# puzzlepaint/camera_calibration

Measured on AMD Instinct MI355X. Metric: M observations/sec per LM iteration, higher is better.
Workload: dtype f64

## Files before the change

camera_calibration_amd/csrc/kernels_obs.hip:

```cpp
#include "cba_internal.h"
#include <algorithm>
#include <mutex>

namespace cba {

__device__ __forceinline__ void quat_mul(const double* a, const double* b, double* o) {
  o[0] = a[0] * b[0] - a[1] * b[1] - a[2] * b[2] - a[3] * b[3];
  o[1] = a[0] * b[1] + a[1] * b[0] + a[2] * b[3] - a[3] * b[2];
  o[2] = a[0] * b[2] + a[2] * b[0] + a[3] * b[1] - a[1] * b[3];
  o[3] = a[0] * b[3] + a[3] * b[0] + a[1] * b[2] - a[2] * b[1];
}
__device__ __forceinline__ void quat_rotate(const double* q, const double* v, double* o) {
  double ux = 2 * (q[2] * v[2] - q[3] * v[1]);
  double uy = 2 * (q[3] * v[0] - q[1] * v[2]);
  double uz = 2 * (q[1] * v[1] - q[2] * v[0]);
  o[0] = v[0] + q[0] * ux + (q[2] * uz - q[3] * uy);
  o[1] = v[1] + q[0] * uy + (q[3] * ux - q[1] * uz);
  o[2] = v[2] + q[0] * uz + (q[1] * uy - q[2] * ux);
}
__device__ __forceinline__ void quat_to_matrix(const double* q, double* R) {
  double tx = 2 * q[1], ty = 2 * q[2], tz = 2 * q[3];
  double twx = tx * q[0], twy = ty * q[0], twz = tz * q[0];
  double txx = tx * q[1], txy = ty * q[1], txz = tz * q[1];
  double tyy = ty * q[2], tyz = tz * q[2], tzz = tz * q[3];
// ... 722 lines not shown
  cells[2 * o] = (int)floor(gx) - 1;
  cells[2 * o + 1] = (int)floor(gy) - 1;
  flags[o] = 3;
  return !localize_only;
}
__global__ void __launch_bounds__(256) k_assemble(PassArgs a, int rig_in_state, int localize_only,
                                                  const double* __restrict__ rig7, const double* __restrict__ camrig7,
                                                  int tasks_per_obs, int rec_doubles, const double* __restrict__ pixels,
                                                  uint8_t* __restrict__ flags, const double* __restrict__ fd_out,
                                                  const uint8_t* __restrict__ fd_ok, double* __restrict__ jrec,
                                                  int* __restrict__ cells, uint8_t* __restrict__ fd_slow) {
  const int64_t o = (int64_t)blockIdx.x * blockDim.x + threadIdx.x;
  const bool with_jacobian = assemble_header(a, o, rig_in_state, localize_only, rig7, camrig7, tasks_per_obs, rec_doubles, pixels, flags,
                                             fd_out, fd_ok, jrec, cells);
  if (o < a.n_obs) fd_slow[o] = flags[o] == 1;
  (void)with_jacobian;
}
int launch_assemble(const PassArgs& a, const Layout& L, const DevState& st, int tasks_per_obs, int rec_doubles,
                    const double* pixels, uint8_t* flags, const double* fd_out, const uint8_t* fd_ok, double* jrec,
                    int* cells, uint8_t* fd_slow, hipStream_t s) {
  if (a.n_obs == 0) return CBA_OK;
  hipLaunchKernelGGL(k_assemble, dim3((unsigned)((a.n_obs + 255) / 256)), dim3(256), 0, s, a, L.rig_in_state,
                     L.localize_only, st.rig_tr_global, st.camera_tr_rig, tasks_per_obs, rec_doubles, pixels, flags,
                     fd_out, fd_ok, jrec, cells, fd_slow);
  CBA_HIP(hipGetLastError());
  return CBA_OK;
}

struct AccumLayout {
  int rig_in_state, eliminate_points, localize_only;
  int first_rig_tr_global, first_camera_tr_rig, first_points;
  int block_dof, block_size, dense_dof;
};
static_assert(std::is_trivially_copyable_v<AccumLayout>);

constexpr int kAccChunk = 8;
constexpr int kAccChunkHot = 64;
constexpr int kHotMax = 12;
constexpr int kHotPairs = kHotMax * (kHotMax + 1) / 2;

template <bool DET> struct Acc;
template <> struct Acc<false> {
  typedef double T;
  static __device__ __forceinline__ T from(double v, double) { return v; }
  static __device__ __forceinline__ void add(double* p, T v) { unsafeAtomicAdd(p, v); }
  static __device__ __forceinline__ void add_lds(double* p, T v) { __hip_atomic_fetch_add(p, v, __ATOMIC_RELAXED, __HIP_MEMORY_SCOPE_WORKGROUP); }
  static __device__ __forceinline__ double to_double(T v, double) { return v; }
};
template <> struct Acc<true> {
  typedef long long T;
  static __device__ __forceinline__ T from(double v, double scale) { return __double2ll_rn(v * scale); }
  static __device__ __forceinline__ void add(double* p, T v) { atomicAdd(reinterpret_cast<unsigned long long*>(p), (unsigned long long)v); }
  static __device__ __forceinline__ void add_lds(double* p, T v) {
    __hip_atomic_fetch_add(reinterpret_cast<unsigned long long*>(p), (unsigned long long)v, __ATOMIC_RELAXED, __HIP_MEMORY_SCOPE_WORKGROUP);
  }
  static __device__ __forceinline__ double to_double(T v, double scale) { return (double)v / scale; }
};

template <bool DET>
__device__ __forceinline__ void acc_add_H(const AccumLayout& L, const AccumTargets& T, int row, int col, typename Acc<DET>::T v) {
  if (row < L.block_dof) {
    if (col < L.block_dof) {
      int blk = row / L.block_size;
      int base = blk * L.block_size;
      Acc<DET>::add(T.Dblk + (size_t)blk * L.block_size * L.block_size + (row - base) * L.block_size + (col - base), v);
    } else {
      Acc<DET>::add(T.B + (size_t)row * L.dense_dof + (col - L.block_dof), v);
    }
  } else {
    Acc<DET>::add(T.Hdd + (size_t)(row - L.block_dof) * L.dense_dof + (col - L.block_dof), v);
  }
}
template <bool DET>
__device__ __forceinline__ void acc_add_b(const AccumLayout& L, const AccumTargets& T, int row, typename Acc<DET>::T v) {
  if (row < L.block_dof) Acc<DET>::add(T.bblk + row, v);
  else Acc<DET>::add(T.bd + (row - L.block_dof), v);
}

template <bool DET>
__global__ void __launch_bounds__(256) k_accumulate(PassArgs a, AccumLayout L, int rec_doubles,
                                                    const uint8_t* __restrict__ flags, const double* __restrict__ jrec,
                                                    const int* __restrict__ cells, const uint32_t* __restrict__ pair_tables,
                                                    const int* __restrict__ pair_counts, AccumTargets T,
                                                    const double* __restrict__ det_scale, int points_separate) {
  typedef typename Acc<DET>::T acc_t;
  const double scale = DET ? det_scale[0] : 1.0;
  const double scale_b = DET ? det_scale[1] : 1.0;
  __shared__ double sJ0[4][kMaxCols];
  __shared__ double sJ1[4][kMaxCols];
  __shared__ double sW0[4][kMaxCols];
  __shared__ double sW1[4][kMaxCols];
  __shared__ int sIdx[4][kMaxCols];
  const int lane = threadIdx.x & 63, wv = threadIdx.x >> 6;
  const int chunk = points_separate ? kAccChunkHot : kAccChunk;
  const int64_t o_begin = ((int64_t)blockIdx.x * 4 + wv) * chunk;
  const int nrig = L.rig_in_state ? 6 : 0;
  const int nh = 6 + nrig;
  const int h0 = L.eliminate_points ? 3 : 0;
  const int nhp = nh * (nh + 1) / 2;
  int hs_i[2], hs_k[2];
#pragma unroll
  for (int t = 0; t < 2; ++t) {
    int sidx = lane + 64 * t;
    hs_i[t] = -1; hs_k[t] = -1;
    if (sidx < nhp) {
      int rem = sidx, i = 0;
      while (rem >= nh - i) { rem -= nh - i; ++i; }
      hs_i[t] = i; hs_k[t] = i + rem;
    } else if (sidx < nhp + nh) {
      hs_i[t] = sidx - nhp; hs_k[t] = -2;
    }
  }
  acc_t hot[2] = {0, 0};
  int cur_pose = -1, cur_rig = -1;
  auto flush = [&]() {
    if (cur_pose < 0) return;
#pragma unroll
    for (int t = 0; t < 2; ++t) {
      if (hs_i[t] < 0) continue;
      int row = hs_i[t] < 6 ? cur_pose + hs_i[t] : cur_rig + hs_i[t] - 6;
      if (hs_k[t] == -2) acc_add_b<DET>(L, T, row, hot[t]);
      else acc_add_H<DET>(L, T, row, hs_k[t] < 6 ? cur_pose + hs_k[t] : cur_rig + hs_k[t] - 6, hot[t]);
      hot[t] = 0;
    }
  };
  for (int c = 0; c < chunk; ++c) {
    const int64_t o = o_begin + c;
    if (o >= a.n_obs) break;
    if (flags[o] != 3) continue;
    const int cam = a.obs_camera[o];
    const CamDev cd = a.cams[cam];
    const int per = cd.params_per_point;
    const int Kg = L.localize_only ? 0 : per * 16;
    const int K = 6 + nrig + 3 + Kg;
    const double* rec = jrec + (size_t)o * rec_doubles;
    const double w = rec[2];
    const int pose_idx = L.first_rig_tr_global + 6 * (a.pose_slot ? a.pose_slot[a.obs_image[o]] : a.obs_image[o]);
    const int rig_idx = L.first_camera_tr_rig + 6 * cam;
    const int point_idx = L.first_points + 3 * a.obs_point[o];
    if (pose_idx != cur_pose || rig_idx != cur_rig) {
      flush();
      cur_pose = pose_idx; cur_rig = rig_idx;
    }
    const int cx0 = cells[2 * o], cy0 = cells[2 * o + 1];
    __builtin_amdgcn_wave_barrier();
    const int Ks = points_separate ? nh : K;
    for (int k = lane; k < Ks; k += 64) {
      int idx; double j0, j1;
      int kk = k;
      if (L.eliminate_points) {
        if (kk < 3) { idx = point_idx + kk; j0 = rec[27 + kk]; j1 = rec[30 + kk]; goto done; }
        kk -= 3;
      }
      if (kk < 6) { idx = pose_idx + kk; j0 = rec[3 + kk]; j1 = rec[9 + kk]; goto done; }
      kk -= 6;
      if (nrig) {
        if (kk < 6) { idx = rig_idx + kk; j0 = rec[15 + kk]; j1 = rec[21 + kk]; goto done; }
        kk -= 6;
      }
      if (!L.eliminate_points) {
        if (kk < 3) { idx = point_idx + kk; j0 = rec[27 + kk]; j1 = rec[30 + kk]; goto done; }
        kk -= 3;
      }
      {
        int cell = kk / per, d = kk - cell * per;
        int seq = (cx0 + (cell & 3)) + (cy0 + (cell >> 2)) * cd.gw;
        idx = L.block_dof + grid_column(cd, seq, d);
        j0 = rec[kRecHeader + kk]; j1 = rec[kRecHeader + Kg + kk];
      }
    done:
      sIdx[wv][k] = idx;
      sJ0[wv][k] = j0; sJ1[wv][k] = j1;
      sW0[wv][k] = w * j0; sW1[wv][k] = w * j1;
    }
    __builtin_amdgcn_wave_barrier();
    __builtin_amdgcn_fence(__ATOMIC_RELEASE, "wavefront");
    const double r0 = rec[0], r1 = rec[1];
#pragma unroll
    for (int t = 0; t < 2; ++t) {
      if (hs_i[t] < 0) continue;
      const int i = h0 + hs_i[t];
      if (hs_k[t] == -2) hot[t] += Acc<DET>::from(r0 * sW0[wv][i] + r1 * sW1[wv][i], scale_b);
      else { const int k = h0 + hs_k[t]; hot[t] += Acc<DET>::from(sW0[wv][i] * sJ0[wv][k] + sW1[wv][i] * sJ1[wv][k], scale); }
    }
    if (points_separate) continue;
    for (int k = lane; k < K - Kg; k += 64) {
      if (k >= h0 && k < h0 + nh) continue;
      acc_add_b<DET>(L, T, sIdx[wv][k], Acc<DET>::from(r0 * sW0[wv][k] + r1 * sW1[wv][k], scale_b));
    }
    const int slot = (per == 2) ? 0 : 1;
    const int npairs = pair_counts[slot];
    const uint32_t* table = pair_tables + (size_t)slot * (kMaxCols * (kMaxCols + 1) / 2);
    for (int e = lane; e < npairs; e += 64) {
      uint32_t pr = table[e];
      int i = pr >> 16, k = pr & 0xffff;
      double v = sW0[wv][i] * sJ0[wv][k] + sW1[wv][i] * sJ1[wv][k];
      acc_add_H<DET>(L, T, sIdx[wv][i], sIdx[wv][k], Acc<DET>::from(v, scale));
    }
  }
  flush();
}
constexpr int kPointChunkColsMax = 5120;
constexpr int kPointThreads = 1024;
constexpr int kPointUnroll = 4;
template <bool DET>
__global__ void __launch_bounds__(kPointThreads) k_accumulate_points(PassArgs a, AccumLayout L, int rec_doubles, const uint8_t* __restrict__ flags,
                                                                     const double* __restrict__ jrec, const int* __restrict__ cells,
                                                                     const int* __restrict__ key_start, const int* __restrict__ key_obs,
                                                                     int n_points, int nchunks, int chunk_cols, AccumTargets T,
                                                                     const double* __restrict__ det_scale) {
  typedef typename Acc<DET>::T acc_t;
  constexpr int NT = kPointThreads, NW = kPointThreads / 64, U = kPointUnroll;
  extern __shared__ double s_rows[];
  __shared__ acc_t s_red[NW][27];
  const double scale = DET ? det_scale[0] : 1.0;
  const double scale_b = DET ? det_scale[1] : 1.0;
  const int key = blockIdx.x / nchunks, chunk = blockIdx.x - key * nchunks;
  const int cam = key / n_points, pt = key - cam * n_points;
  const CamDev& cd = a.cams[cam];
  const int per = cd.params_per_point, gw = cd.gw;
  const int* __restrict__ gperm = cd.gperm;
  const int Kg = L.localize_only ? 0 : per * 16;
  const int ncols = Kg ? per * gw * cd.gh : 0;
  const int c0 = chunk * chunk_cols;
  const int o_begin = key_start[key], n = key_start[key + 1] - o_begin;
  if (n == 0 || (chunk > 0 && c0 >= ncols)) return;
  const int c1 = c0 + chunk_cols < ncols ? c0 + chunk_cols : ncols;
  const int tid = threadIdx.x, lane = tid & 63, wv = tid >> 6;
  const int nrig = L.rig_in_state ? 6 : 0;
  const int point_idx = L.first_points + 3 * pt;
  if (c0 < c1) {
    for (int i = tid; i < 3 * chunk_cols; i += NT) s_rows[i] = 0.0;
    __syncthreads();
    const int items = n * Kg;
    for (int it0 = tid; it0 < items; it0 += NT * U) {
      int64_t o[U]; int kk[U]; bool live[U];
#pragma unroll
      for (int u = 0; u < U; ++u) {
        const int it = it0 + u * NT;
        live[u] = it < items;
        const int oi = live[u] ? it / Kg : 0;
        kk[u] = live[u] ? it - oi * Kg : 0;
        o[u] = key_obs[o_begin + oi];
      }
      int cx[U], cy[U]; uint8_t fl[U];
#pragma unroll
      for (int u = 0; u < U; ++u) { fl[u] = flags[o[u]]; cx[u] = cells[2 * o[u]]; cy[u] = cells[2 * o[u] + 1]; }
      int col[U];
#pragma unroll
      for (int u = 0; u < U; ++u) {
        const int cell = kk[u] / per, d = kk[u] - cell * per;
        int seq = (cx[u] + (cell & 3)) + (cy[u] + (cell >> 2)) * gw;
        live[u] = live[u] && fl[u] == 3;
        if (!live[u]) seq = 0;
        col[u] = per * (gperm ? gperm[seq] : seq) + d;
        live[u] = live[u] && col[u] >= c0 && col[u] < c1;
      }
      double w[U], g0[U], g1[U], q0[U][3], q1[U][3];
#pragma unroll
      for (int u = 0; u < U; ++u) {
        if (!live[u]) continue;
        const double* rec = jrec + (size_t)o[u] * rec_doubles;
        w[u] = rec[2]; g0[u] = rec[kRecHeader + kk[u]]; g1[u] = rec[kRecHeader + Kg + kk[u]];
#pragma unroll
        for (int r = 0; r < 3; ++r) { q0[u][r] = rec[27 + r]; q1[u][r] = rec[30 + r]; }
      }
#pragma unroll
      for (int u = 0; u < U; ++u) {
        if (!live[u]) continue;
#pragma unroll
        for (int r = 0; r < 3; ++r)
          Acc<DET>::add_lds(&s_rows[r * chunk_cols + (col[u] - c0)], Acc<DET>::from((w[u] * q0[u][r]) * g0[u] + (w[u] * q1[u][r]) * g1[u], scale));
      }
    }
    __syncthreads();
#pragma unroll
    for (int r = 0; r < 3; ++r) {
      double* out = T.Hdd + (size_t)(point_idx - L.block_dof + r) * L.dense_dof + cd.intr_offset + c0;
      for (int c = tid; c < c1 - c0; c += NT) out[c] = s_rows[r * chunk_cols + c];
    }
// ... 185 lines not shown
#pragma unroll 1
    for (int r = 0; r < nrec; ++r) {
      const double w = sW[r];
      if (tid < KG) bacc += Acc<DET>::from(sRes[r][0] * (w * sJ0[r][tid]) + sRes[r][1] * (w * sJ1[r][tid]), scale_b);
      if (has_tile) {
        double a0[TZ], a1[TZ], b0[TZ], b1[TZ];
#pragma unroll
        for (int x = 0; x < TZ; ++x) { a0[x] = sJ0[r][i0 + x]; a1[x] = sJ1[r][i0 + x]; b0[x] = sJ0[r][k0 + x]; b1[x] = sJ1[r][k0 + x]; }
#pragma unroll
        for (int x = 0; x < TZ; ++x)
#pragma unroll
          for (int y = 0; y < TZ; ++y) acc[x][y] += Acc<DET>::from(w * (a0[x] * b0[y] + a1[x] * b1[y]), scale);
      }
      if (rig) {
#pragma unroll
        for (int t = 0; t < NR; ++t) {
          const int e = tid + 256 * t;
          if (e < 6 * KG) { const int q = e / KG, k = e - q * KG; racc[t] += Acc<DET>::from(w * (sRig[r][q] * sJ0[r][k] + sRig[r][6 + q] * sJ1[r][k]), scale); }
        }
      }
    }
  }
  const CamDev cd = a.cams[cam];
  const int cy0 = cell / cd.gw, cx0 = cell - cy0 * cd.gw;
  if (tid < KG) {
    const int ck = tid / PER, dk = tid - ck * PER;
    Acc<DET>::add(bd + grid_column(cd, (cx0 + (ck & 3)) + (cy0 + (ck >> 2)) * cd.gw, dk), bacc);
  }
  if (has_tile) {
#pragma unroll
    for (int x = 0; x < TZ; ++x)
#pragma unroll
      for (int y = 0; y < TZ; ++y) {
        const int i = i0 + x, k = k0 + y;
        if (i > k) continue;
        const int ci = i / PER, di = i - ci * PER, ck = k / PER, dk = k - ck * PER;
        int row = grid_column(cd, (cx0 + (ci & 3)) + (cy0 + (ci >> 2)) * cd.gw, di);
        int col = grid_column(cd, (cx0 + (ck & 3)) + (cy0 + (ck >> 2)) * cd.gw, dk);
        if (row > col) { const int t2 = row; row = col; col = t2; }
        Acc<DET>::add(Hdd + (size_t)row * ld + col, acc[x][y]);
      }
  }
  if (!rig) return;
#pragma unroll
  for (int t = 0; t < NR; ++t) {
    const int e = tid + 256 * t;
    if (e >= 6 * KG) continue;
    const int q = e / KG, k = e - q * KG, ck = k / PER, dk = k - ck * PER;
    const int col = grid_column(cd, (cx0 + (ck & 3)) + (cy0 + (ck >> 2)) * cd.gw, dk);
    Acc<DET>::add(Hdd + (size_t)(rig_row0 + q) * ld + col, racc[t]);
  }
}
int launch_accumulate_cells(const PassArgs& a, const std::vector<cba_camera>& cams, const std::vector<int>& cell_base_host,
                            int rec_doubles, int ld, const uint8_t* flags, const double* jrec, const int* cells,
                            const int* cell_base, int* count, int* start, int* fill, int* order, double* Hdd,
                            int rig_row_first , const double* det_scale, double* bd,
                            hipStream_t s) {
  if (a.n_obs == 0) return CBA_OK;
  const int n_keys = cell_base_host.back();
  CBA_HIP(hipMemsetAsync(count, 0, sizeof(int) * (size_t)n_keys, s));
  CBA_HIP(hipMemsetAsync(fill, 0, sizeof(int) * (size_t)n_keys, s));
  dim3 grid((unsigned)((a.n_obs + 255) / 256)), block(256);
  hipLaunchKernelGGL(k_cell_count, grid, block, 0, s, a, flags, cells, cell_base, count);
  hipLaunchKernelGGL(k_cell_scan, dim3(1), dim3(1024), 0, s, count, n_keys, start);
  hipLaunchKernelGGL(k_cell_fill, grid, block, 0, s, a, flags, cells, cell_base, start, fill, order);
  for (size_t c = 0; c < cams.size(); ++c) {
    const int n_cells = cams[c].grid_w * cams[c].grid_h;
    dim3 g2((unsigned)n_cells);
    const int rr = rig_row_first >= 0 ? rig_row_first + 6 * (int)c : -1;
    const bool central = cams[c].model_type == CBA_CENTRAL_GENERIC;
#define CBA_CELLS2(PER_, DET_, RIG_) hipLaunchKernelGGL((k_accumulate_cells<PER_, DET_, RIG_>), g2, block, 0, s, a, (int)c, cell_base_host[c], \
                                                        n_cells, rec_doubles, ld, jrec, start, order, Hdd, rr, det_scale, bd)
#define CBA_CELLS(PER_, DET_) do { if (rr >= 0) CBA_CELLS2(PER_, DET_, true); else CBA_CELLS2(PER_, DET_, false); } while (0)
    if (central) { if (det_scale) CBA_CELLS(2, true); else CBA_CELLS(2, false); }
    else { if (det_scale) CBA_CELLS(5, true); else CBA_CELLS(5, false); }
#undef CBA_CELLS2
#undef CBA_CELLS
  }
  CBA_HIP(hipGetLastError());
  return CBA_OK;
}

constexpr int kStripBand = 1024;
__global__ void __launch_bounds__(256) k_strip_band_mask(PassArgs a, AccumLayout L, const uint8_t* __restrict__ flags,
                                                         const int* __restrict__ cells, unsigned long long* __restrict__ band_mask, int n_bands) {
  const int64_t o = (int64_t)blockIdx.x * blockDim.x + threadIdx.x;
  if (o >= a.n_obs) return;
  if (flags[o] != 3) { band_mask[o] = 0ull; return; }
  if (n_bands > 64) { band_mask[o] = ~0ull; return; }
  const CamDev cd = a.cams[a.obs_camera[o]];
  unsigned long long m = 0ull;
  const int pc = L.first_points - L.block_dof + 3 * a.obs_point[o];
  m |= 1ull << (pc / kStripBand); m |= 1ull << ((pc + 2) / kStripBand);
  if (!L.localize_only) {
    const int cx0 = cells[2 * o], cy0 = cells[2 * o + 1];
    for (int c = 0; c < 16; ++c) {
      const int col = grid_column(cd, (cx0 + (c & 3)) + (cy0 + (c >> 2)) * cd.gw, 0);
      m |= 1ull << (col / kStripBand); m |= 1ull << ((col + cd.params_per_point - 1) / kStripBand);
    }
  }
  band_mask[o] = m;
}
constexpr int kStripWaves = 8;
template <bool DET>
__global__ void __launch_bounds__(64 * kStripWaves) k_accumulate_strips(PassArgs a, AccumLayout L, int rec_doubles, const uint8_t* __restrict__ flags,
                                                            const double* __restrict__ jrec, const int* __restrict__ cells,
                                                            const unsigned long long* __restrict__ band_mask,
                                                            const int64_t* __restrict__ img_start, double* __restrict__ B, int ld,
                                                            const double* __restrict__ det_scale) {
  __shared__ double acc[6][kStripBand];
  const double scale = DET ? *det_scale : 1.0;
  const int img = blockIdx.x, band = blockIdx.y;
  const int col_lo = band * kStripBand;
  const int col_hi = min(col_lo + kStripBand, ld);
  for (int i = threadIdx.x; i < 6 * kStripBand; i += 64 * kStripWaves) (&acc[0][0])[i] = 0.0;
  __syncthreads();
  const int lane = threadIdx.x & 63, wv = threadIdx.x >> 6;
  const unsigned long long bit = 1ull << (band & 63);
  const int64_t o_begin = img_start[img], o_end = img_start[img + 1];
  __shared__ unsigned long long gmask[kStripWaves];
  for (int64_t p0 = o_begin; p0 < o_end; p0 += 64 * kStripWaves) {
    const int64_t mine = p0 + 64 * wv + lane;
    const bool hit = mine < o_end && (band_mask[mine] & bit);
    const unsigned long long bal = __ballot(hit);
    if (lane == 0) gmask[wv] = bal;
    __syncthreads();
    int seen = 0;
    for (int gidx = 0; gidx < kStripWaves; ++gidx) {
      unsigned long long todo = gmask[gidx];
      while (todo) {
        const int idx = __builtin_ctzll(todo);
        todo &= todo - 1;
        if (((seen++) % kStripWaves) != wv) continue;
        const int64_t o = p0 + 64 * gidx + idx;
        const CamDev cd = a.cams[a.obs_camera[o]];
        const int per = cd.params_per_point;
        const int Kg = L.localize_only ? 0 : per * 16;
        const int nc = 3 + Kg;
        const double* rec = jrec + (size_t)o * rec_doubles;
        const int cx0 = cells[2 * o], cy0 = cells[2 * o + 1];
        const int point_col = L.first_points - L.block_dof + 3 * a.obs_point[o];
        const double w = rec[2];
        for (int c = lane; c < nc; c += 64) {
          int col; double j0, j1;
          if (c < 3) { col = point_col + c; j0 = rec[27 + c]; j1 = rec[30 + c]; }
          else {
            const int g = c - 3, cell = g / per, d = g - cell * per;
            col = grid_column(cd, (cx0 + (cell & 3)) + (cy0 + (cell >> 2)) * cd.gw, d);
            j0 = rec[kRecHeader + g]; j1 = rec[kRecHeader + Kg + g];
          }
          if (col < col_lo || col >= col_hi) continue;
          const double w0 = w * j0, w1 = w * j1;
#pragma unroll
          for (int k = 0; k < 6; ++k) Acc<DET>::add(&acc[k][col - col_lo], Acc<DET>::from(rec[3 + k] * w0 + rec[9 + k] * w1, scale));
        }
      }
    }
    __syncthreads();
  }
  __syncthreads();
  const int slot = a.pose_slot ? a.pose_slot[img] : img;
  for (int k = 0; k < 6; ++k) {
    double* row = B + (size_t)(6 * slot + k) * ld + col_lo;
    for (int c = threadIdx.x; c < col_hi - col_lo; c += 64 * kStripWaves) row[c] = acc[k][c];
  }
}
int launch_accumulate_strips(const PassArgs& a, const Layout& L, int n_images, int rec_doubles, const uint8_t* flags, const double* jrec,
                             const int* cells, unsigned long long* band_mask, const int64_t* img_start, double* B, int ld, const double* det_scale,
                             hipStream_t s) {
  if (n_images == 0) return CBA_OK;
  AccumLayout al;
  al.rig_in_state = L.rig_in_state; al.eliminate_points = L.eliminate_points; al.localize_only = L.localize_only;
  al.first_rig_tr_global = L.first_rig_tr_global; al.first_camera_tr_rig = L.first_camera_tr_rig;
  al.first_points = L.first_points; al.block_dof = L.block_dof; al.block_size = L.block_size; al.dense_dof = L.dense_dof;
  const int bands = (ld + kStripBand - 1) / kStripBand;
  if (a.n_obs > 0)
    hipLaunchKernelGGL(k_strip_band_mask, dim3((unsigned)((a.n_obs + 255) / 256)), dim3(256), 0, s, a, al, flags, cells, band_mask, bands);
  if (det_scale)
    hipLaunchKernelGGL(k_accumulate_strips<true>, dim3((unsigned)n_images, (unsigned)bands), dim3(64 * kStripWaves), 0, s, a, al, rec_doubles, flags,
                       jrec, cells, band_mask, img_start, B, ld, det_scale);
  else
    hipLaunchKernelGGL(k_accumulate_strips<false>, dim3((unsigned)n_images, (unsigned)bands), dim3(64 * kStripWaves), 0, s, a, al, rec_doubles, flags,
                       jrec, cells, band_mask, img_start, B, ld, det_scale);
  CBA_HIP(hipGetLastError());
  return CBA_OK;
}

int launch_accumulate(const PassArgs& a, const Layout& L, int rec_doubles, const uint8_t* flags, const double* jrec,
                      const int* cells, const uint32_t* pair_tables, const int* pair_counts, AccumTargets t,
                      const double* det_scale, int points_separate, hipStream_t s) {
  if (a.n_obs == 0) return CBA_OK;
  AccumLayout al;
  al.rig_in_state = L.rig_in_state; al.eliminate_points = L.eliminate_points; al.localize_only = L.localize_only;
  al.first_rig_tr_global = L.first_rig_tr_global; al.first_camera_tr_rig = L.first_camera_tr_rig;
  al.first_points = L.first_points; al.block_dof = L.block_dof; al.block_size = L.block_size; al.dense_dof = L.dense_dof;
  const int chunk = points_separate ? kAccChunkHot : kAccChunk;
  const dim3 grid((unsigned)((a.n_obs + 4 * chunk - 1) / (4 * chunk)));
  if (det_scale)
    hipLaunchKernelGGL(k_accumulate<true>, grid, dim3(256), 0, s, a, al, rec_doubles, flags, jrec, cells, pair_tables, pair_counts, t, det_scale, points_separate);
  else
    hipLaunchKernelGGL(k_accumulate<false>, grid, dim3(256), 0, s, a, al, rec_doubles, flags, jrec, cells, pair_tables, pair_counts, t, det_scale, points_separate);
  CBA_HIP(hipGetLastError());
  return CBA_OK;
}

__global__ void __launch_bounds__(256) k_det_bound(int64_t n, int rec_doubles, int used_doubles, const uint8_t* __restrict__ flags,
                                                   const double* __restrict__ jrec, unsigned long long* __restrict__ out_bits) {
  const int lane = threadIdx.x & 63;
  double m = 0.0, mb = 0.0;
  for (int64_t o = (int64_t)blockIdx.x * 4 + (threadIdx.x >> 6); o < n; o += (int64_t)gridDim.x * 4) {
    if (flags[o] != 3) continue;
    const double* rec = jrec + (size_t)o * rec_doubles;
    double jm = 0.0;
    for (int k = lane; k < used_doubles; k += 64) if (k > 2) jm = fmax(jm, fabs(rec[k]));
    for (int off = 32; off > 0; off >>= 1) jm = fmax(jm, __shfl_xor(jm, off, 64));
    m = fmax(m, 2.0 * rec[2] * jm * jm);
    mb = fmax(mb, 2.0 * rec[2] * jm * fmax(fabs(rec[0]), fabs(rec[1])));
  }
  if (lane == 0 && m > 0.0) atomicMax(out_bits, (unsigned long long)__double_as_longlong(m));
  if (lane == 0 && mb > 0.0) atomicMax(out_bits + 1, (unsigned long long)__double_as_longlong(mb));
}
__global__ void k_det_scale(const unsigned long long* __restrict__ bits, int64_t n_obs, double* __restrict__ scale) {
  for (int i = 0; i < 2; ++i) {
    const double m = __longlong_as_double((long long)bits[i]);
    const double bound = m * (double)(n_obs > 0 ? n_obs : 1);
    int e = 0;
    if (bound > 0.0) frexp(bound, &e);
    scale[i] = ldexp(1.0, 62 - e);
  }
}
int launch_det_scale(int64_t n, int rec_doubles, int used_doubles, const uint8_t* flags, const double* jrec, unsigned long long* bits,
                     double* scale, hipStream_t s) {
  CBA_HIP(hipMemsetAsync(bits, 0, 2 * sizeof(unsigned long long), s));
  if (n > 0) hipLaunchKernelGGL(k_det_bound, dim3(1024), dim3(256), 0, s, n, rec_doubles, used_doubles, flags, jrec, bits);
  hipLaunchKernelGGL(k_det_scale, dim3(1), dim3(1), 0, s, bits, n, scale);
  CBA_HIP(hipGetLastError());
  return CBA_OK;
}
__global__ void __launch_bounds__(256) k_det_convert(double* __restrict__ p, size_t n, const double* __restrict__ det_scale) {
  const double inv = 1.0 / *det_scale;
  for (size_t i = (size_t)blockIdx.x * 256 + threadIdx.x; i < n; i += (size_t)gridDim.x * 256)
    p[i] = (double)(*reinterpret_cast<const long long*>(p + i)) * inv;
}
int launch_det_convert(double* p, size_t n, const double* det_scale, hipStream_t s) {
  if (n == 0) return CBA_OK;
  const size_t blocks = (n + 255) / 256;
  hipLaunchKernelGGL(k_det_convert, dim3((unsigned)(blocks < 65536 ? blocks : 65536)), dim3(256), 0, s, p, n, det_scale);
  CBA_HIP(hipGetLastError());
  return CBA_OK;
}

constexpr int kRedBlocks = 256;
__global__ void __launch_bounds__(256) k_reduce_costs_partial(const double* __restrict__ ref, const double* __restrict__ test,
                                                              const uint8_t* __restrict__ flags, int64_t n,
                                                              double* __restrict__ partials) {
  double acc[8] = {0, 0, 0, 0, 0, 0, 0, 0};
  for (int64_t i = (int64_t)blockIdx.x * 256 + threadIdx.x; i < n; i += (int64_t)kRedBlocks * 256) {
    double r = ref ? ref[i] : -1.0, t = test ? test[i] : -1.0;
    if (r >= 0) { acc[0] += r; acc[5] += 1; }
    if (t >= 0) { acc[1] += t; acc[6] += 1; }
    if (r >= 0 && t >= 0) { acc[2] += r; acc[3] += t; acc[4] += 1; }
    if (flags && flags[i] == 1) acc[7] += 1;
  }
  __shared__ double sh[8][256];
#pragma unroll
  for (int k = 0; k < 8; ++k) sh[k][threadIdx.x] = acc[k];
  __syncthreads();
  for (int s = 128; s > 0; s >>= 1) {
    if ((int)threadIdx.x < s)
#pragma unroll
      for (int k = 0; k < 8; ++k) sh[k][threadIdx.x] += sh[k][threadIdx.x + s];
    __syncthreads();
  }
  if (threadIdx.x < 8) partials[blockIdx.x * 8 + threadIdx.x] = sh[threadIdx.x][0];
}
__global__ void k_reduce_costs_final(const double* __restrict__ partials, double* __restrict__ out8) {
  int k = threadIdx.x;
  if (k >= 8) return;
  double s = 0;
  for (int b = 0; b < kRedBlocks; ++b) s += partials[b * 8 + k];
  out8[k] = s;
}
int launch_reduce_costs(const double* ref, const double* test, const uint8_t* flags, int64_t n, double* partials,
                        double* out8, hipStream_t s) {
// ... 145 lines not shown
```

Before: 32.59.

## Split pose accumulation into staged kernel and restructure strip accumulation work distribution

Adds a dedicated k_accumulate_poses kernel for the points-separate path. It stages record headers and pose/rig indices for 32 observations per wavefront in shared memory and reads the pose Jacobians directly, with no per-column scatter. The strip accumulation kernel is restructured in two ways: point columns get their own pass where each lane handles one coordinate of one observation, and grid columns are spread evenly over flattened (observation, column) items using a prefix-compacted hit list and shuffle-broadcast headers. Camera parameters are cached in shared memory, and the band-mask kernel is skipped in localize-only mode. The goal is to cut serial per-observation loops and poor lane utilization, at the cost of more complex indexing and extra unrolled loads.

```diff
diff --git a/camera_calibration_amd/csrc/kernels_obs.hip b/camera_calibration_amd/csrc/kernels_obs.hip
--- a/camera_calibration_amd/csrc/kernels_obs.hip
+++ b/camera_calibration_amd/csrc/kernels_obs.hip
@@ -828,7 +828,7 @@
                                                     const uint8_t* __restrict__ flags, const double* __restrict__ jrec,
                                                     const int* __restrict__ cells, const uint32_t* __restrict__ pair_tables,
                                                     const int* __restrict__ pair_counts, AccumTargets T,
-                                                    const double* __restrict__ det_scale, int points_separate) {
+                                                    const double* __restrict__ det_scale) {
   typedef typename Acc<DET>::T acc_t;
   const double scale = DET ? det_scale[0] : 1.0;
   const double scale_b = DET ? det_scale[1] : 1.0;
@@ -838,8 +838,7 @@
   __shared__ double sW1[4][kMaxCols];
   __shared__ int sIdx[4][kMaxCols];
   const int lane = threadIdx.x & 63, wv = threadIdx.x >> 6;
-  const int chunk = points_separate ? kAccChunkHot : kAccChunk;
-  const int64_t o_begin = ((int64_t)blockIdx.x * 4 + wv) * chunk;
+  const int64_t o_begin = ((int64_t)blockIdx.x * 4 + wv) * kAccChunk;
   const int nrig = L.rig_in_state ? 6 : 0;
   const int nh = 6 + nrig;
   const int h0 = L.eliminate_points ? 3 : 0;
@@ -870,7 +869,7 @@
       hot[t] = 0;
     }
   };
-  for (int c = 0; c < chunk; ++c) {
+  for (int c = 0; c < kAccChunk; ++c) {
     const int64_t o = o_begin + c;
     if (o >= a.n_obs) break;
     if (flags[o] != 3) continue;
@@ -890,8 +889,7 @@
     }
     const int cx0 = cells[2 * o], cy0 = cells[2 * o + 1];
     __builtin_amdgcn_wave_barrier();
-    const int Ks = points_separate ? nh : K;
-    for (int k = lane; k < Ks; k += 64) {
+    for (int k = lane; k < K; k += 64) {
       int idx; double j0, j1;
       int kk = k;
       if (L.eliminate_points) {
@@ -929,7 +927,6 @@
       if (hs_k[t] == -2) hot[t] += Acc<DET>::from(r0 * sW0[wv][i] + r1 * sW1[wv][i], scale_b);
       else { const int k = h0 + hs_k[t]; hot[t] += Acc<DET>::from(sW0[wv][i] * sJ0[wv][k] + sW1[wv][i] * sJ1[wv][k], scale); }
     }
-    if (points_separate) continue;
     for (int k = lane; k < K - Kg; k += 64) {
       if (k >= h0 && k < h0 + nh) continue;
       acc_add_b<DET>(L, T, sIdx[wv][k], Acc<DET>::from(r0 * sW0[wv][k] + r1 * sW1[wv][k], scale_b));
@@ -942,6 +939,89 @@
       int i = pr >> 16, k = pr & 0xffff;
       double v = sW0[wv][i] * sJ0[wv][k] + sW1[wv][i] * sJ1[wv][k];
       acc_add_H<DET>(L, T, sIdx[wv][i], sIdx[wv][k], Acc<DET>::from(v, scale));
+    }
+  }
+  flush();
+}
+constexpr int kPoseStage = 32;
+static_assert(kAccChunkHot % kPoseStage == 0, "a wavefront's chunk is a whole number of stages");
+template <bool DET, bool RIG>
+__global__ void __launch_bounds__(256) k_accumulate_poses(PassArgs a, AccumLayout L, int rec_doubles, const uint8_t* __restrict__ flags,
+                                                          const double* __restrict__ jrec, AccumTargets T, const double* __restrict__ det_scale) {
+  typedef typename Acc<DET>::T acc_t;
+  constexpr int NH = RIG ? 12 : 6;
+  constexpr int NHP = NH * (NH + 1) / 2;
+  constexpr int ND = RIG ? 27 : 15;
+  constexpr int SLOTS = (NHP + NH + 63) / 64;
+  const double scale = DET ? det_scale[0] : 1.0;
+  const double scale_b = DET ? det_scale[1] : 1.0;
+  __shared__ double s_hdr[4][kPoseStage][ND];
+  __shared__ int s_pose[4][kPoseStage], s_rig[4][kPoseStage];
+  const int lane = threadIdx.x & 63, wv = threadIdx.x >> 6;
+  const int64_t o_begin = ((int64_t)blockIdx.x * 4 + wv) * kAccChunkHot;
+  int hs_i[SLOTS], hs_k[SLOTS];
+#pragma unroll
+  for (int t = 0; t < SLOTS; ++t) {
+    const int sidx = lane + 64 * t;
+    hs_i[t] = -1; hs_k[t] = -1;
+    if (sidx < NHP) {
+      int rem = sidx, i = 0;
+      while (rem >= NH - i) { rem -= NH - i; ++i; }
+      hs_i[t] = i; hs_k[t] = i + rem;
+    } else if (sidx < NHP + NH) {
+      hs_i[t] = sidx - NHP; hs_k[t] = -2;
+    }
+  }
+  acc_t hot[SLOTS];
+#pragma unroll
+  for (int t = 0; t < SLOTS; ++t) hot[t] = 0;
+  int cur_pose = -1, cur_rig = -1;
+  auto flush = [&]() {
+    if (cur_pose < 0) return;
+#pragma unroll
+    for (int t = 0; t < SLOTS; ++t) {
+      if (hs_i[t] < 0) continue;
+      const int row = hs_i[t] < 6 ? cur_pose + hs_i[t] : cur_rig + hs_i[t] - 6;
+      if (hs_k[t] == -2) acc_add_b<DET>(L, T, row, hot[t]);
+      else acc_add_H<DET>(L, T, row, hs_k[t] < 6 ? cur_pose + hs_k[t] : cur_rig + hs_k[t] - 6, hot[t]);
+      hot[t] = 0;
+    }
+  };
+  for (int st = 0; st < kAccChunkHot; st += kPoseStage) {
+    const int64_t o0 = o_begin + st;
+    if (o0 >= a.n_obs) break;
+    const int nst = (int)(a.n_obs - o0 < kPoseStage ? a.n_obs - o0 : kPoseStage);
+    __builtin_amdgcn_wave_barrier();
+    if (lane < nst) {
+      const int64_t o = o0 + lane;
+      const int img = a.obs_image[o];
+      s_pose[wv][lane] = flags[o] == 3 ? L.first_rig_tr_global + 6 * (a.pose_slot ? a.pose_slot[img] : img) : -1;
+      s_rig[wv][lane] = L.first_camera_tr_rig + 6 * a.obs_camera[o];
+    }
+    for (int idx = lane; idx < nst * ND; idx += 64) {
+      const int c = idx / ND, k = idx - c * ND;
+      s_hdr[wv][c][k] = jrec[(size_t)(o0 + c) * rec_doubles + k];
+    }
+    __builtin_amdgcn_wave_barrier();
+    __builtin_amdgcn_fence(__ATOMIC_RELEASE, "wavefront");
+    for (int c = 0; c < nst; ++c) {
+      const int pose_idx = __builtin_amdgcn_readfirstlane(s_pose[wv][c]);
+      if (pose_idx < 0) continue;
+      const int rig_idx = __builtin_amdgcn_readfirstlane(s_rig[wv][c]);
+      if (pose_idx != cur_pose || rig_idx != cur_rig) {
+        flush();
+        cur_pose = pose_idx; cur_rig = rig_idx;
+      }
+      const double* h = s_hdr[wv][c];
+      const double r0 = h[0], r1 = h[1], w = h[2];
+#pragma unroll
+      for (int t = 0; t < SLOTS; ++t) {
+        if (hs_i[t] < 0) continue;
+        const int i = hs_i[t], k = hs_k[t];
+        const double w0 = w * h[(i < 6 ? 3 : 9) + i], w1 = w * h[(i < 6 ? 9 : 15) + i];
+        if (k == -2) hot[t] += Acc<DET>::from(r0 * w0 + r1 * w1, scale_b);
+        else hot[t] += Acc<DET>::from(w0 * h[(k < 6 ? 3 : 9) + k] + w1 * h[(k < 6 ? 9 : 15) + k], scale);
+      }
     }
   }
   flush();
@@ -1293,7 +1373,7 @@
 }
 
 constexpr int kStripBand = 1024;
-__global__ void __launch_bounds__(256) k_strip_band_mask(PassArgs a, AccumLayout L, const uint8_t* __restrict__ flags,
+__global__ void __launch_bounds__(256) k_strip_band_mask(PassArgs a, const uint8_t* __restrict__ flags,
                                                          const int* __restrict__ cells, unsigned long long* __restrict__ band_mask, int n_bands) {
   const int64_t o = (int64_t)blockIdx.x * blockDim.x + threadIdx.x;
   if (o >= a.n_obs) return;
@@ -1301,73 +1381,148 @@
   if (n_bands > 64) { band_mask[o] = ~0ull; return; }
   const CamDev cd = a.cams[a.obs_camera[o]];
   unsigned long long m = 0ull;
-  const int pc = L.first_points - L.block_dof + 3 * a.obs_point[o];
-  m |= 1ull << (pc / kStripBand); m |= 1ull << ((pc + 2) / kStripBand);
-  if (!L.localize_only) {
-    const int cx0 = cells[2 * o], cy0 = cells[2 * o + 1];
-    for (int c = 0; c < 16; ++c) {
-      const int col = grid_column(cd, (cx0 + (c & 3)) + (cy0 + (c >> 2)) * cd.gw, 0);
-      m |= 1ull << (col / kStripBand); m |= 1ull << ((col + cd.params_per_point - 1) / kStripBand);
-    }
+  const int cx0 = cells[2 * o], cy0 = cells[2 * o + 1];
+  for (int c = 0; c < 16; ++c) {
+    const int col = grid_column(cd, (cx0 + (c & 3)) + (cy0 + (c >> 2)) * cd.gw, 0);
+    m |= 1ull << (col / kStripBand); m |= 1ull << ((col + cd.params_per_point - 1) / kStripBand);
   }
   band_mask[o] = m;
 }
 constexpr int kStripWaves = 8;
+constexpr int kStripPointGroup = 21;
+constexpr int kStripUnroll = 2;
+constexpr int kStripTripObs = 2;
+static_assert(kMaxGridCols == 80, "k_accumulate_strips: a wavefront trip is assumed to cover at most kStripTripObs observations");
 template <bool DET>
-__global__ void __launch_bounds__(64 * kStripWaves) k_accumulate_strips(PassArgs a, AccumLayout L, int rec_doubles, const uint8_t* __restrict__ flags,
+__global__ void __launch_bounds__(64 * kStripWaves) k_accumulate_strips(PassArgs a, AccumLayout L, int n_points, int rec_doubles,
+                                                            const uint8_t* __restrict__ flags,
                                                             const double* __restrict__ jrec, const int* __restrict__ cells,
                                                             const unsigned long long* __restrict__ band_mask,
                                                             const int64_t* __restrict__ img_start, double* __restrict__ B, int ld,
                                                             const double* __restrict__ det_scale) {
+  constexpr int U = kStripUnroll, G = kStripPointGroup;
   __shared__ double acc[6][kStripBand];
+  __shared__ int s_per[kMaxCameras], s_gw[kMaxCameras], s_off[kMaxCameras];
+  __shared__ const int* s_perm[kMaxCameras];
   const double scale = DET ? *det_scale : 1.0;
   const int img = blockIdx.x, band = blockIdx.y;
   const int col_lo = band * kStripBand;
   const int col_hi = min(col_lo + kStripBand, ld);
   for (int i = threadIdx.x; i < 6 * kStripBand; i += 64 * kStripWaves) (&acc[0][0])[i] = 0.0;
+  if (threadIdx.x < a.n_cameras) {
+    const CamDev& cd = a.cams[threadIdx.x];
+    s_per[threadIdx.x] = cd.params_per_point; s_gw[threadIdx.x] = cd.gw; s_off[threadIdx.x] = cd.intr_offset; s_perm[threadIdx.x] = cd.gperm;
+  }
   __syncthreads();
   const int lane = threadIdx.x & 63, wv = threadIdx.x >> 6;
+  const int64_t o_begin = img_start[img], o_end = img_start[img + 1];
+
+  const int pt_lo = L.first_points - L.block_dof, pt_hi = pt_lo + 3 * n_points;
+  if (col_lo < pt_hi && pt_lo < col_hi) {
+    const int j = lane / 3, c = lane - 3 * j;
+    const int64_t ntrips = (o_end - o_begin + G - 1) / G;
+    for (int64_t t0 = wv; t0 < ntrips; t0 += kStripWaves * U) {
+      int64_t o[U]; bool live[U];
+#pragma unroll
+      for (int u = 0; u < U; ++u) {
+        o[u] = o_begin + (t0 + u * kStripWaves) * G + j;
+        live[u] = j < G && o[u] < o_end;
+        if (!live[u]) o[u] = o_begin;
+      }
+      uint8_t fl[U]; int pt[U];
+#pragma unroll
+      for (int u = 0; u < U; ++u) { fl[u] = flags[o[u]]; pt[u] = a.obs_point[o[u]]; }
+      int col[U];
+#pragma unroll
+      for (int u = 0; u < U; ++u) {
+        col[u] = pt_lo + 3 * pt[u] + c;
+        live[u] = live[u] && fl[u] == 3 && col[u] >= col_lo && col[u] < col_hi;
+      }
+      double w[U], j0[U], j1[U], h0[U][6], h1[U][6];
+#pragma unroll
+      for (int u = 0; u < U; ++u) {
+        if (!live[u]) continue;
+        const double* rec = jrec + (size_t)o[u] * rec_doubles;
+        w[u] = rec[2]; j0[u] = rec[27 + c]; j1[u] = rec[30 + c];
+#pragma unroll
+        for (int k = 0; k < 6; ++k) { h0[u][k] = rec[3 + k]; h1[u][k] = rec[9 + k]; }
+      }
+#pragma unroll
+      for (int u = 0; u < U; ++u) {
+        if (!live[u]) continue;
+        const double w0 = w[u] * j0[u], w1 = w[u] * j1[u];
+#pragma unroll
+        for (int k = 0; k < 6; ++k) Acc<DET>::add(&acc[k][col[u] - col_lo], Acc<DET>::from(h0[u][k] * w0 + h1[u][k] * w1, scale));
+      }
+    }
+  }
+
+  int kslot = 0;
+  if (!L.localize_only)
+    for (int cam = 0; cam < a.n_cameras; ++cam) kslot = max(kslot, 16 * s_per[cam]);
+  __shared__ unsigned long long gmask[kStripWaves];
+  __shared__ unsigned short s_list[64 * kStripWaves];
   const unsigned long long bit = 1ull << (band & 63);
-  const int64_t o_begin = img_start[img], o_end = img_start[img + 1];
-  __shared__ unsigned long long gmask[kStripWaves];
-  for (int64_t p0 = o_begin; p0 < o_end; p0 += 64 * kStripWaves) {
+  const int hl = lane >> 4, he = lane & 15;
+  for (int64_t p0 = o_begin; kslot > 0 && p0 < o_end; p0 += 64 * kStripWaves) {
     const int64_t mine = p0 + 64 * wv + lane;
     const bool hit = mine < o_end && (band_mask[mine] & bit);
     const unsigned long long bal = __ballot(hit);
     if (lane == 0) gmask[wv] = bal;
     __syncthreads();
-    int seen = 0;
-    for (int gidx = 0; gidx < kStripWaves; ++gidx) {
-      unsigned long long todo = gmask[gidx];
-      while (todo) {
-        const int idx = __builtin_ctzll(todo);
-        todo &= todo - 1;
-        if (((seen++) % kStripWaves) != wv) continue;
-        const int64_t o = p0 + 64 * gidx + idx;
-        const CamDev cd = a.cams[a.obs_camera[o]];
-        const int per = cd.params_per_point;
-        const int Kg = L.localize_only ? 0 : per * 16;
-        const int nc = 3 + Kg;
-        const double* rec = jrec + (size_t)o * rec_doubles;
-        const int cx0 = cells[2 * o], cy0 = cells[2 * o + 1];
-        const int point_col = L.first_points - L.block_dof + 3 * a.obs_point[o];
-        const double w = rec[2];
-        for (int c = lane; c < nc; c += 64) {
-          int col; double j0, j1;
-          if (c < 3) { col = point_col + c; j0 = rec[27 + c]; j1 = rec[30 + c]; }
-          else {
-            const int g = c - 3, cell = g / per, d = g - cell * per;
-            col = grid_column(cd, (cx0 + (cell & 3)) + (cy0 + (cell >> 2)) * cd.gw, d);
-            j0 = rec[kRecHeader + g]; j1 = rec[kRecHeader + Kg + g];
-          }
-          if (col < col_lo || col >= col_hi) continue;
-          const double w0 = w * j0, w1 = w * j1;
-#pragma unroll
-          for (int k = 0; k < 6; ++k) Acc<DET>::add(&acc[k][col - col_lo], Acc<DET>::from(rec[3 + k] * w0 + rec[9 + k] * w1, scale));
-        }
-      }
-    }
+    int before = 0, total = 0;
+    for (int g = 0; g < kStripWaves; ++g) {
+      const int n = __popcll(gmask[g]);
+      if (g < wv) before += n;
+      total += n;
+    }
+    if (hit) s_list[before + __popcll(bal & ((1ull << lane) - 1ull))] = (unsigned short)(64 * wv + lane);
     __syncthreads();
+    const int items = total * kslot;
+    for (int f0 = 64 * wv; f0 < items; f0 += 64 * kStripWaves * U) {
+      int64_t o[U], oh[U]; int g[U], src[U]; bool live[U], hlive[U];
+#pragma unroll
+      for (int u = 0; u < U; ++u) {
+        const int first = f0 + u * 64 * kStripWaves, f = first + lane;
+        live[u] = f < items;
+        const int m = live[u] ? f / kslot : 0;
+        g[u] = f - m * kslot;
+        o[u] = p0 + s_list[m];
+        const int mh = first / kslot + hl;
+        hlive[u] = first < items && hl < kStripTripObs && he < 13 && mh < total;
+        oh[u] = p0 + s_list[hlive[u] ? mh : 0];
+        src[u] = live[u] ? 16 * (m - first / kslot) : 0;
+      }
+      int cam[U], cx[U], cy[U]; double hv[U];
+#pragma unroll
+      for (int u = 0; u < U; ++u) {
+        cam[u] = a.obs_camera[o[u]]; cx[u] = cells[2 * o[u]]; cy[u] = cells[2 * o[u] + 1];
+        hv[u] = hlive[u] ? jrec[(size_t)oh[u] * rec_doubles + 2 + he] : 0.0;
+      }
+      int col[U]; double j0[U], j1[U];
+#pragma unroll
+      for (int u = 0; u < U; ++u) {
+        const int per = s_per[cam[u]], Kg = 16 * per, gg = g[u];
+        live[u] = live[u] && gg < Kg;
+        const int cell = live[u] ? gg / per : 0, d = live[u] ? gg - cell * per : 0;
+        const int seq = (cx[u] + (cell & 3)) + (cy[u] + (cell >> 2)) * s_gw[cam[u]];
+        const int* perm = s_perm[cam[u]];
+        col[u] = s_off[cam[u]] + per * (perm ? perm[seq] : seq) + d;
+        const double* rec = jrec + (size_t)o[u] * rec_doubles + kRecHeader;
+        j0[u] = live[u] ? rec[gg] : 0.0; j1[u] = live[u] ? rec[Kg + gg] : 0.0;
+      }
+#pragma unroll
+      for (int u = 0; u < U; ++u) {
+        const double w = __shfl(hv[u], src[u], 64);
+        double h0[6], h1[6];
+#pragma unroll
+        for (int k = 0; k < 6; ++k) { h0[k] = __shfl(hv[u], src[u] + 1 + k, 64); h1[k] = __shfl(hv[u], src[u] + 7 + k, 64); }
+        if (!live[u] || col[u] < col_lo || col[u] >= col_hi) continue;
+        const double w0 = w * j0[u], w1 = w * j1[u];
+#pragma unroll
+        for (int k = 0; k < 6; ++k) Acc<DET>::add(&acc[k][col[u] - col_lo], Acc<DET>::from(h0[k] * w0 + h1[k] * w1, scale));
+      }
+    }
   }
   __syncthreads();
   const int slot = a.pose_slot ? a.pose_slot[img] : img;
@@ -1385,13 +1540,13 @@
   al.first_rig_tr_global = L.first_rig_tr_global; al.first_camera_tr_rig = L.first_camera_tr_rig;
   al.first_points = L.first_points; al.block_dof = L.block_dof; al.block_size = L.block_size; al.dense_dof = L.dense_dof;
   const int bands = (ld + kStripBand - 1) / kStripBand;
-  if (a.n_obs > 0)
-    hipLaunchKernelGGL(k_strip_band_mask, dim3((unsigned)((a.n_obs + 255) / 256)), dim3(256), 0, s, a, al, flags, cells, band_mask, bands);
+  if (a.n_obs > 0 && !L.localize_only)
+    hipLaunchKernelGGL(k_strip_band_mask, dim3((unsigned)((a.n_obs + 255) / 256)), dim3(256), 0, s, a, flags, cells, band_mask, bands);
   if (det_scale)
-    hipLaunchKernelGGL(k_accumulate_strips<true>, dim3((unsigned)n_images, (unsigned)bands), dim3(64 * kStripWaves), 0, s, a, al, rec_doubles, flags,
+    hipLaunchKernelGGL(k_accumulate_strips<true>, dim3((unsigned)n_images, (unsigned)bands), dim3(64 * kStripWaves), 0, s, a, al, L.n_points, rec_doubles, flags,
                        jrec, cells, band_mask, img_start, B, ld, det_scale);
   else
-    hipLaunchKernelGGL(k_accumulate_strips<false>, dim3((unsigned)n_images, (unsigned)bands), dim3(64 * kStripWaves), 0, s, a, al, rec_doubles, flags,
+    hipLaunchKernelGGL(k_accumulate_strips<false>, dim3((unsigned)n_images, (unsigned)bands), dim3(64 * kStripWaves), 0, s, a, al, L.n_points, rec_doubles, flags,
                        jrec, cells, band_mask, img_start, B, ld, det_scale);
   CBA_HIP(hipGetLastError());
   return CBA_OK;
@@ -1407,10 +1562,15 @@
   al.first_points = L.first_points; al.block_dof = L.block_dof; al.block_size = L.block_size; al.dense_dof = L.dense_dof;
   const int chunk = points_separate ? kAccChunkHot : kAccChunk;
   const dim3 grid((unsigned)((a.n_obs + 4 * chunk - 1) / (4 * chunk)));
-  if (det_scale)
-    hipLaunchKernelGGL(k_accumulate<true>, grid, dim3(256), 0, s, a, al, rec_doubles, flags, jrec, cells, pair_tables, pair_counts, t, det_scale, points_separate);
+#define CBA_POSES(DET_, RIG_) hipLaunchKernelGGL((k_accumulate_poses<DET_, RIG_>), grid, dim3(256), 0, s, a, al, rec_doubles, flags, jrec, t, det_scale)
+  if (points_separate) {
+    if (det_scale) { if (L.rig_in_state) CBA_POSES(true, true); else CBA_POSES(true, false); }
+    else { if (L.rig_in_state) CBA_POSES(false, true); else CBA_POSES(false, false); }
+  } else if (det_scale)
+    hipLaunchKernelGGL(k_accumulate<true>, grid, dim3(256), 0, s, a, al, rec_doubles, flags, jrec, cells, pair_tables, pair_counts, t, det_scale);
   else
-    hipLaunchKernelGGL(k_accumulate<false>, grid, dim3(256), 0, s, a, al, rec_doubles, flags, jrec, cells, pair_tables, pair_counts, t, det_scale, points_separate);
+    hipLaunchKernelGGL(k_accumulate<false>, grid, dim3(256), 0, s, a, al, rec_doubles, flags, jrec, cells, pair_tables, pair_counts, t, det_scale);
+#undef CBA_POSES
   CBA_HIP(hipGetLastError());
   return CBA_OK;
 }
```

Result: faster. 34.11, median of 6 (+4.7%).
